# jmschrei/PyPore

Hardware: AMD Instinct MI355X
Metric: Msamples/sec segmented (SpeedyStatSplit, 10^8-sample trace); %HBM roofline (higher is better)
Workload: dtype int32/f64 (exact integer block sums of fp32 or int16 samples; decisions in fp64)

## Files before the change

### pypore_amd/csrc/seg_bs.hpp

```cpp
#pragma once
#include <type_traits>

namespace ps {

constexpr int BS_WIDE = 16384;
enum : unsigned { ST_WIDE_RANGE = 16u };
constexpr int BS_CHUNK = 128;
constexpr int BS_CHUNK_LOG = 7;
constexpr int BS_MAXCH = 64;
constexpr int BSW_LIM = 1 << 23;
template <int DT> constexpr bool bs_wide() { return (DT & DT_WIDE) != 0; }
__device__ __forceinline__ long long i64_of(int lo, int hi) { return (static_cast<long long>(hi) << 32) | static_cast<unsigned>(lo); }
__device__ __forceinline__ double d_of_i64(long long x)
{
    return fma(static_cast<double>(static_cast<int>(x >> 32)), 4294967296.0, static_cast<double>(static_cast<unsigned>(x)));
}
__device__ __forceinline__ unsigned long long u64_of(unsigned lo, unsigned hi) { return (static_cast<unsigned long long>(hi) << 32) | lo; }
__device__ __forceinline__ int bs8_s1(uint2 v) { return static_cast<int>(v.y) >> 7; }
__device__ __forceinline__ unsigned long long bs8_s2(uint2 v) { return u64_of(v.x, v.y & 0x7fu); }
__device__ __forceinline__ double bs8_s2_biased(uint2 v) { return __hiloint2double(static_cast<int>((v.y & 0x7fu) | 0x43300000u), static_cast<int>(v.x)); }
constexpr double BS_BIAS = 4503599627370496.0;
__device__ __forceinline__ uint2 bs8_pack(int e1, unsigned long long e2)
{
    return make_uint2(static_cast<unsigned>(e2), (static_cast<unsigned>(e1) << 7) | static_cast<unsigned>(e2 >> 32));
// ... 93 lines not shown
constexpr int BS_GRP_SAMPLES = 8 * BS_GRP;
#define PS_OCT_STEPS(X) X(0xB1) X(0x4E) X(0x141)
__device__ __forceinline__ int oct_allsum(int x)
{
#define PS_STEP(CTRL) { x += dpp_mov<CTRL, 0xf>(0, x); }
    PS_OCT_STEPS(PS_STEP)
#undef PS_STEP
    return x;
}
__device__ __forceinline__ int oct_allmax(int x)
{
#define PS_STEP(CTRL) { x = max(x, dpp_mov<CTRL, 0xf>(static_cast<int>(0x80000000), x)); }
    PS_OCT_STEPS(PS_STEP)
#undef PS_STEP
    return x;
}
__device__ __forceinline__ int oct_allmin(int x)
{
#define PS_STEP(CTRL) { x = min(x, dpp_mov<CTRL, 0xf>(0x7fffffff, x)); }
    PS_OCT_STEPS(PS_STEP)
#undef PS_STEP
    return x;
}
__device__ __forceinline__ float oct_allmaxf(float x)
{
#define PS_STEP(CTRL) { x = __uint_as_float(max(__float_as_uint(x), static_cast<unsigned>(dpp_mov<CTRL, 0xf>(0, static_cast<int>(__float_as_uint(x)))))); }
    PS_OCT_STEPS(PS_STEP)
#undef PS_STEP
    return x;
}
__device__ __forceinline__ float pmaxf(float a, float b) { return __int_as_float(max(__float_as_int(a), __float_as_int(b))); }
__device__ __forceinline__ int oct_first(int x, int lane)
{
    const int q = __builtin_amdgcn_update_dpp(0, x, 0x00, 0xf, 0xf, true);
    const int s = __builtin_amdgcn_update_dpp(0, q, 0x114, 0xf, 0xf, true);
    return (lane & 4) ? s : q;
}

#ifndef PS_K0_AMP
#define PS_K0_AMP 2
#endif
#ifndef PS_K0_TRIM
#define PS_K0_TRIM 1
#endif
#ifndef PS_K0_MINW
#define PS_K0_MINW 4
#endif
constexpr int K0_BPT = 4;
constexpr int K0_WB = 64 * K0_BPT;
#ifndef PS_K0_WAVES
#define PS_K0_WAVES 4
#endif
#ifndef PS_K0_PKF32
#define PS_K0_PKF32 1
#endif
#ifndef PS_K0_PK16
#define PS_K0_PK16 1
#endif
#ifndef PS_K0_PRIO
#define PS_K0_PRIO 0
#endif
constexpr int K0_WAVES = PS_K0_WAVES;
__host__ __device__ inline long long k0_padded_blocks(long long nb_total) { return (nb_total + 1 + K0_WB - 1) / K0_WB * K0_WB; }

__device__ __forceinline__ void k0_lds_ready() { asm volatile("s_waitcnt lgkmcnt(0)" ::: "memory"); __builtin_amdgcn_wave_barrier(); }
__device__ __forceinline__ void k0_lds_done() { __builtin_amdgcn_wave_barrier(); asm volatile("" ::: "memory"); }

template <int DT> struct K0Rec { int s1; unsigned s2; unsigned long long s2w; int ymin, ymax; };
template <int DT> struct K0Gen { K0Rec<DT> r; int m; unsigned bad; };

template <int DT>
__device__ __forceinline__ void k0_block_sums(const int (&y)[8], K0Rec<DT> &r)
{
    constexpr bool WIDE = bs_wide<DT>();
    r.s1 = 0; r.s2 = 0; r.s2w = 0;
#pragma unroll
    for (int q = 0; q < 8; ++q) {
        r.s1 += y[q];
        if constexpr (WIDE) r.s2w += static_cast<unsigned long long>(static_cast<long long>(y[q]) * static_cast<long long>(y[q]));
#if !PS_K0_TRIM
        else r.s2 += static_cast<unsigned>(__mul24(y[q], y[q]));
#endif
    }
#if PS_K0_TRIM
    if constexpr (!WIDE) {
        unsigned acc = static_cast<unsigned>(__mul24(y[0], y[0]));
#pragma unroll
        for (int q = 1; q < 8; ++q) asm("v_mad_i32_i24 %0, %1, %1, %2" : "=v"(acc) : "v"(y[q]), "v"(acc));
        r.s2 = acc;
    }
#endif
    r.ymin = min(min(min(y[0], y[1]), min(y[2], y[3])), min(min(y[4], y[5]), min(y[6], y[7])));
    r.ymax = max(max(max(y[0], y[1]), max(y[2], y[3])), max(max(y[4], y[5]), max(y[6], y[7])));
}

template <int DT>
__device__ __forceinline__ void k0_offsets(const DevCfg &c, const int4 *raw, int m, float mf, unsigned &nz, int (&y)[8])
{
    if (sdt(DT) == PS_DTYPE_F32) {
        const f2 iq = {c.inv_q, c.inv_q};
        const f2 mf2 = {mf, mf};
#pragma unroll
        for (int v = 0; v < 2; ++v) {
#pragma clang fp contract(off)
            const int w[4] = {raw[v].x, raw[v].y, raw[v].z, raw[v].w};
#pragma unroll
            for (int h = 0; h < 2; ++h) {
                const f2 x = {__int_as_float(w[2 * h]), __int_as_float(w[2 * h + 1])};
                const f2 t = x * iq;
                const f2 r = {__builtin_rintf(t.x), __builtin_rintf(t.y)};
                const f2 d = t - r;
                nz |= __float_as_uint(d.x) | __float_as_uint(d.y);
                const f2 yf = r - mf2;
                y[v * 4 + 2 * h] = static_cast<int>(yf.x);
                y[v * 4 + 2 * h + 1] = static_cast<int>(yf.y);
            }
        }
    } else {
        const int w[4] = {raw[0].x, raw[0].y, raw[0].z, raw[0].w};
        const int om = c.off_counts - m;
#pragma unroll
        for (int q = 0; q < 8; ++q)
            y[q] = ((q & 1) ? (w[q >> 1] >> 16) : static_cast<int>(static_cast<short>(w[q >> 1] & 0xffff))) + om;
    }
}

typedef short k0_v2s __attribute__((ext_vector_type(2)));
__device__ __forceinline__ int k0_dot2_first(k0_v2s a, k0_v2s b)
{
    int out;
    asm("v_dot2_i32_i16 %0, %1, %2, 0" : "=v"(out) : "v"(a), "v"(b));
    return out;
}

template <int DT>
__device__ __forceinline__ void k0_block_sums_pk16(const int4 raw, int k0pk, K0Rec<DT> &r)
{
    const k0_v2s k0v = __builtin_bit_cast(k0_v2s, k0pk);
    const k0_v2s ones = {1, 1};
    const int w[4] = {raw.x, raw.y, raw.z, raw.w};
    k0_v2s y[4];
    int s1 = 0, s2 = 0;
#pragma unroll
    for (int q = 0; q < 4; ++q) {
        y[q] = __builtin_elementwise_sub_sat(__builtin_bit_cast(k0_v2s, w[q]), k0v);
        s1 = q == 0 ? k0_dot2_first(y[q], ones) : __builtin_amdgcn_sdot2(y[q], ones, s1, false);
        s2 = q == 0 ? k0_dot2_first(y[q], y[q]) : __builtin_amdgcn_sdot2(y[q], y[q], s2, false);
    }
    const k0_v2s mn = __builtin_elementwise_min(__builtin_elementwise_min(y[0], y[1]), __builtin_elementwise_min(y[2], y[3]));
    const k0_v2s mx = __builtin_elementwise_max(__builtin_elementwise_max(y[0], y[1]), __builtin_elementwise_max(y[2], y[3]));
    r.s1 = s1; r.s2 = static_cast<unsigned>(s2); r.s2w = 0;
    r.ymin = min(static_cast<int>(mn.x), static_cast<int>(mn.y));
    r.ymax = max(static_cast<int>(mx.x), static_cast<int>(mx.y));
}

template <int DT>
__device__ __forceinline__ void k0_block_sums_pkf32(const int4 (&raw)[2], float inv_q, float mf, unsigned &nz, K0Rec<DT> &r)
{
    const f2 iq = {inv_q, inv_q}, m2 = {mf, mf};
    const f2 cn = {1.0f / 32767.0f, 1.0f / 32767.0f};
    const k0_v2s ones = {1, 1};
    const int w[8] = {raw[0].x, raw[0].y, raw[0].z, raw[0].w, raw[1].x, raw[1].y, raw[1].z, raw[1].w};
    k0_v2s y[4];
    int s1 = 0, s2 = 0;
#pragma unroll
    for (int h = 0; h < 4; ++h) {
#pragma clang fp contract(off)
        const f2 x = {__int_as_float(w[2 * h]), __int_as_float(w[2 * h + 1])};
        const f2 t = x * iq;
        nz |= __float_as_uint(__builtin_amdgcn_fractf(t.x)) | __float_as_uint(__builtin_amdgcn_fractf(t.y));
        const f2 a = (t - m2) * cn;
        y[h] = __builtin_amdgcn_cvt_pknorm_i16(a.x, a.y);
        s1 = h == 0 ? k0_dot2_first(y[h], ones) : __builtin_amdgcn_sdot2(y[h], ones, s1, false);
        s2 = h == 0 ? k0_dot2_first(y[h], y[h]) : __builtin_amdgcn_sdot2(y[h], y[h], s2, false);
    }
    const k0_v2s mn = __builtin_elementwise_min(__builtin_elementwise_min(y[0], y[1]), __builtin_elementwise_min(y[2], y[3]));
    const k0_v2s mx = __builtin_elementwise_max(__builtin_elementwise_max(y[0], y[1]), __builtin_elementwise_max(y[2], y[3]));
    r.s1 = s1; r.s2 = static_cast<unsigned>(s2); r.s2w = 0;
    r.ymin = min(static_cast<int>(mn.x), static_cast<int>(mn.y));
    r.ymax = max(static_cast<int>(mx.x), static_cast<int>(mx.y));
}

template <int DT>
__device__ __attribute__((noinline)) K0Gen<DT> k0_block_general(BsCold k, const int64_t *ev_start, const int64_t *ev_len, const int64_t *ev_boff,
                                                                int64_t n_samples, long long gb, long long nb_total, int e_hint, int4 *ev_info)
{
    const DevCfg c = bs_cold_cfg(k);
    K0Gen<DT> out;
    K0Rec<DT> &r = out.r;
    unsigned bad = 0;
    r.s1 = 0; r.s2 = 0; r.s2w = 0; r.ymin = 0; r.ymax = 0;
    out.m = 0; out.bad = 0;
    if (gb >= nb_total) return out;
    int e = e_hint;
    while (ev_boff[e + 1] <= gb) ++e;
    const int64_t len = ev_len[e], base = ev_start[e];
    const long long b = gb - ev_boff[e];
    const int64_t i0 = 8 * b;
    const int m = load_count<DT>(c, base, bad);
    out.m = m;
    int y[8];
    const int cnt = static_cast<int>(len - i0 < 8 ? len - i0 : 8);
    constexpr int ES = static_cast<int>(sizeof(typename Raw<DT>::type));
    const char *p = static_cast<const char *>(c.samples) + (base + i0) * ES;
    if (cnt == 8 && (reinterpret_cast<uintptr_t>(p) & 15u) == 0) {
        constexpr int NV = 8 * ES / 16;
        int4 raw[2];
#pragma unroll
        for (int v = 0; v < NV; ++v) raw[v] = reinterpret_cast<const int4 *>(p)[v];
        unsigned nz = 0;
        k0_offsets<DT>(c, raw, m, static_cast<float>(m), nz, y);
        if (nz) bad |= ST_OFF_GRID;
        k0_block_sums<DT>(y, r);
    } else if (sdt(DT) == PS_DTYPE_I16 && cnt == 8 && base + i0 >= 1 && base + i0 + 10 <= n_samples) {
        const uintptr_t a = reinterpret_cast<uintptr_t>(p);
        const int *q4 = reinterpret_cast<const int *>(a & ~static_cast<uintptr_t>(3));
        int v[5];
#pragma unroll
        for (int q = 0; q < 5; ++q) v[q] = q4[q];
        const bool odd = (a & 2u) != 0;
        const int om = c.off_counts - m;
#pragma unroll
        for (int q = 0; q < 4; ++q) {
            const int w = odd ? static_cast<int>((static_cast<unsigned>(v[q]) >> 16) | (static_cast<unsigned>(v[q + 1]) << 16)) : v[q];
            y[2 * q] = static_cast<int>(static_cast<short>(w & 0xffff)) + om;
            y[2 * q + 1] = (w >> 16) + om;
        }
        k0_block_sums<DT>(y, r);
    } else {
#pragma unroll
        for (int q = 0; q < 8; ++q) y[q] = q < cnt ? load_count<DT>(c, base + i0 + q, bad) - m : 0;
        k0_block_sums<DT>(y, r);
        r.ymin = r.ymax = y[0];
#pragma unroll
        for (int q = 1; q < 8; ++q)
            if (q < cnt) { r.ymin = min(r.ymin, y[q]); r.ymax = max(r.ymax, y[q]); }
    }
    if (b == 0) ev_info[e] = make_int4(m, 0, static_cast<int>(ev_boff[e] & 0xffffffffLL), static_cast<int>(ev_boff[e] >> 32));
    out.bad = bad;
    return out;
}

struct K0Src { int e; int fast; long long b_first; int64_t base; };
template <int A> struct K0Vec;
template <> struct K0Vec<2> { typedef int type __attribute__((ext_vector_type(4), aligned(2))); };
template <> struct K0Vec<4> { typedef int type __attribute__((ext_vector_type(4), aligned(4))); };
template <int A> __device__ __forceinline__ int4 k0_load16(const char *p)
{
    const typename K0Vec<A>::type v = *reinterpret_cast<const typename K0Vec<A>::type *>(p);
    return make_int4(v.x, v.y, v.z, v.w);
}
template <int A>
__global__ void k0_unaligned_probe_kernel(const unsigned char *buf, int n_off, unsigned *bad)
{
    const int o = threadIdx.x;
    if (o >= n_off) return;
    const int4 v = k0_load16<A>(reinterpret_cast<const char *>(buf) + o * A);
    const unsigned char *q = buf + o * A;
    unsigned w[4];
    for (int k = 0; k < 4; ++k) w[k] = q[4 * k] | (q[4 * k + 1] << 8) | (q[4 * k + 2] << 16) | (static_cast<unsigned>(q[4 * k + 3]) << 24);
    if (static_cast<unsigned>(v.x) != w[0] || static_cast<unsigned>(v.y) != w[1] || static_cast<unsigned>(v.z) != w[2] || static_cast<unsigned>(v.w) != w[3])
        atomicOr(bad, 1u);
}

template <int DT, int NS = 2>
__global__ __launch_bounds__(64 * K0_WAVES, (NS > 2 ? 2 : PS_K0_MINW)) void blocksum_kernel(DevCfg c, const int64_t *__restrict__ ev_start, const int64_t *__restrict__ ev_len,
                                                                const int64_t *__restrict__ ev_boff, int n_ev, int64_t n_samples, void *bs_out,
                                                                int4 *ev_info, int4 *chunk_tot, unsigned *status, uint4 *grp_out)
{
    constexpr bool WIDE = bs_wide<DT>();
    constexpr int LIM = WIDE ? BSW_LIM : BS_WIDE;
    constexpr int ES = static_cast<int>(sizeof(typename Raw<DT>::type));
    constexpr int NV = 8 * ES / 16;
    __shared__ int4 tr[K0_WAVES][K0_WB];
    const int lane = threadIdx.x & 63;
    const int wave = uni(static_cast<int>(threadIdx.x >> 6));
    const long long nwv = static_cast<long long>(gridDim.x) * K0_WAVES;
    long long wv = static_cast<long long>(blockIdx.x) * K0_WAVES + wave;
    const long long nb_total = ev_boff[n_ev];
    const long long n_wb = nb_total / K0_WB + 1;
    if (wv >= n_wb) return;
#if PS_K0_PRIO
    __builtin_amdgcn_s_setprio(PS_K0_PRIO);
#endif
    unsigned bad = 0;
    int4 *mine = tr[wave];
    auto classify = [&](long long wb0, int e_lo) -> K0Src {
        K0Src s;
        const long long gfirst = min(wb0, nb_total - 1);
        int lo = e_lo, hi = n_ev - 1;
        while (lo < hi) {
            const int mid = (lo + hi + 1) >> 1;
            if (ev_boff[mid] <= gfirst) lo = mid; else hi = mid - 1;
        }
        s.e = lo;
        s.b_first = wb0 - ev_boff[lo];
        s.base = ev_start[lo];
        const int64_t len_f = ev_len[lo];
        s.fast = wb0 + K0_WB <= ev_boff[lo + 1] && 8 * (s.b_first + K0_WB) <= len_f && nb_total > 0;
        if (!c.k0_unaligned && ((reinterpret_cast<uintptr_t>(c.samples) + static_cast<uintptr_t>((s.base + 8 * s.b_first) * ES)) & 15u) != 0) s.fast = 0;
        return s;
    };
    using raw_t = typename Raw<DT>::type;
    auto issue = [&](const K0Src &s, int4 (&raw)[K0_BPT][NV], raw_t &first) {
        const char *pb = s.fast ? static_cast<const char *>(c.samples) + (s.base + 8 * s.b_first) * ES : static_cast<const char *>(bs_out);
        first = *reinterpret_cast<const raw_t *>(s.fast ? static_cast<const char *>(c.samples) + s.base * ES : static_cast<const char *>(bs_out));
        const unsigned lo = static_cast<unsigned>(lane) * (8u * ES);
#pragma unroll
        for (int k = 0; k < K0_BPT; ++k)
#pragma unroll
            for (int v = 0; v < NV; ++v) raw[k][v] = k0_load16<ES>(pb + (lo + static_cast<unsigned>(k * 64 * 8 * ES + 16 * v)));
    };
    auto process = [&](auto fast_tag, const long long wb0, const K0Src &src, const int4 (&raw)[K0_BPT][NV], const raw_t first) {
    constexpr bool FAST = decltype(fast_tag)::value;
    const int e_first = src.e;
    int ymn_all = 0x7fffffff, ymx_all = -0x7fffffff - 1;
    auto put = [&](int k, const K0Rec<DT> &r) {
        if (PS_K0_TRIM) { ymn_all = min(ymn_all, r.ymin); ymx_all = max(ymx_all, r.ymax); }
        else if (r.ymax >= LIM || r.ymin <= -LIM) bad |= ST_WIDE_RANGE;
        if constexpr (WIDE) mine[64 * k + lane] = make_int4(r.s1, max(-r.ymin, r.ymax), static_cast<int>(r.s2w), static_cast<int>(r.s2w >> 32));
        else mine[64 * k + lane] = make_int4(r.s1, static_cast<int>(r.s2), (r.ymin & 0xffff) | (r.ymax << 16), 0);
    };
    if constexpr (FAST) {
        const int m = to_count<DT>(c, first, bad);
        const float mf = static_cast<float>(m);
        unsigned nz = 0;
        const bool look = sdt(DT) == PS_DTYPE_F32 && (WIDE || m > 8388607 - LIM || m < -8388607 + LIM);
        constexpr bool PK16 = sdt(DT) == PS_DTYPE_I16 && !WIDE && PS_K0_PK16;
        const int k0raw = m - c.off_counts;
        const int k0pk = (k0raw & 0xffff) | (k0raw << 16);
#pragma unroll
        for (int k = 0; k < K0_BPT; ++k) {
            int y[8];
            K0Rec<DT> r;
            if constexpr (PK16) {
                k0_block_sums_pk16<DT>(raw[k][0], k0pk, r);
            } else if constexpr (sdt(DT) == PS_DTYPE_F32 && !WIDE && PS_K0_PKF32) {
                k0_block_sums_pkf32<DT>(raw[k], c.inv_q, mf, nz, r);
                asm volatile("" : "+v"(nz));
            } else {
            k0_offsets<DT>(c, raw[k], m, mf, nz, y);
            asm volatile("" : "+v"(nz));
            k0_block_sums<DT>(y, r);
            }
            if (!PS_K0_TRIM && look) {
                const int ka = m + r.ymin, kb = m + r.ymax;
                if (max(ka < 0 ? -ka : ka, kb < 0 ? -kb : kb) >= 8388608) bad |= ST_OFF_GRID;
            }
            put(k, r);
            __builtin_amdgcn_sched_barrier(0);
        }
        if (PS_K0_TRIM && look) {
            const int ka = m + ymn_all, kb = m + ymx_all;
            if (max(ka < 0 ? -ka : ka, kb < 0 ? -kb : kb) >= 8388608) bad |= ST_OFF_GRID;
        }
        if (nz) bad |= ST_OFF_GRID;
        if (src.b_first + lane == 0) ev_info[e_first] = make_int4(m, 0, static_cast<int>(ev_boff[e_first] & 0xffffffffLL), static_cast<int>(ev_boff[e_first] >> 32));
    } else {
#pragma unroll 1
        for (int k = 0; k < K0_BPT; ++k) {
            const K0Gen<DT> g = k0_block_general<DT>(bs_cold(c), ev_start, ev_len, ev_boff, n_samples, wb0 + 64 * k + lane, nb_total, e_first, ev_info);
            bad |= g.bad;
            if (sdt(DT) == PS_DTYPE_F32) {
                const int ka = g.m + g.r.ymin, kb = g.m + g.r.ymax;
                if (max(ka < 0 ? -ka : ka, kb < 0 ? -kb : kb) >= 8388608) bad |= ST_OFF_GRID;
            }
            put(k, g.r);
        }
    }
    if (PS_K0_TRIM && (ymx_all >= LIM || ymn_all <= -LIM)) bad |= ST_WIDE_RANGE;
    k0_lds_ready();
    int4 t[K0_BPT];
#pragma unroll
    for (int j = 0; j < K0_BPT; ++j) t[j] = mine[K0_BPT * lane + j];
    const long long gb4 = wb0 + K0_BPT * lane;
    const long long chunk = (wb0 >> BS_CHUNK_LOG) + (lane >> 5);
    if constexpr (WIDE) {
        long long e1[K0_BPT], e2[K0_BPT];
        long long r1 = 0, r2 = 0;
        int yabs = 0;
#pragma unroll
        for (int j = 0; j < K0_BPT; ++j) {
            e1[j] = r1; e2[j] = r2;
            r1 += t[j].x; r2 += i64_of(t[j].z, t[j].w);
            yabs = max(yabs, t[j].y);
        }
        const long long i1 = half_incl_scan_i64(r1), i2 = half_incl_scan_i64(r2);
        const long long x1 = i1 - r1, x2 = i2 - r2;
        int4 *bs = static_cast<int4 *>(bs_out) + gb4;
#pragma unroll
        for (int j = 0; j < K0_BPT; ++j) {
            const long long a1 = x1 + e1[j], a2 = x2 + e2[j];
            bs[j] = make_int4(static_cast<int>(a1), static_cast<int>(a1 >> 32), static_cast<int>(a2), static_cast<int>(a2 >> 32));
        }
        yabs = half_max_i32(yabs);
        if ((lane & 31) == 31) {
            chunk_tot[2 * chunk] = make_int4(static_cast<int>(i1), static_cast<int>(i1 >> 32), static_cast<int>(i2), static_cast<int>(i2 >> 32));
            chunk_tot[2 * chunk + 1] = make_int4(yabs, 0, 0, 0);
        }
    } else {
        int e1[K0_BPT];
        unsigned long long e2[K0_BPT];
        int r1 = 0;
        unsigned long long r2 = 0;
#pragma unroll
        for (int j = 0; j < K0_BPT; ++j) {
            e1[j] = r1; e2[j] = r2;
            r1 += t[j].x; r2 += static_cast<unsigned>(t[j].y);
        }
        const int mmn = min(min(static_cast<int>(static_cast<short>(t[0].z & 0xffff)), static_cast<int>(static_cast<short>(t[1].z & 0xffff))),
                            min(static_cast<int>(static_cast<short>(t[2].z & 0xffff)), static_cast<int>(static_cast<short>(t[3].z & 0xffff))));
        const int mmx = max(max(t[0].z >> 16, t[1].z >> 16), max(t[2].z >> 16, t[3].z >> 16));
        int yabs = max(-mmn, mmx);
        const int i1 = half_incl_scan_i32(r1);
        const int r2lo = static_cast<int>(r2 & 0xffffu), r2hi = static_cast<int>(r2 >> 16);
        const int ilo = half_incl_scan_i32(r2lo), ihi = half_incl_scan_i32(r2hi);
        const int x1 = i1 - r1;
        const unsigned long long x2 = (static_cast<unsigned long long>(static_cast<unsigned>(ihi - r2hi)) << 16) + static_cast<unsigned>(ilo - r2lo);
        uint2 ent[K0_BPT];
#pragma unroll
        for (int j = 0; j < K0_BPT; ++j) ent[j] = bs8_pack(x1 + e1[j], x2 + e2[j]);
        uint4 *bs = reinterpret_cast<uint4 *>(static_cast<uint2 *>(bs_out) + gb4);
        bs[0] = make_uint4(ent[0].x, ent[0].y, ent[1].x, ent[1].y);
        bs[1] = make_uint4(ent[2].x, ent[2].y, ent[3].x, ent[3].y);
        if (c.blk_mm) *reinterpret_cast<int4 *>(c.blk_mm + gb4) = make_int4(t[0].z, t[1].z, t[2].z, t[3].z);
        if (c.blk_cls) {
            unsigned b2 = 0;
            const int ythr = c.cls_kthr - load_count<DT>(c, ev_start[0], b2);
            unsigned cb = 0;
            int cmn = 0x7fffffff, cmx = -0x7fffffff;
#pragma unroll
            for (int j = 0; j < K0_BPT; ++j) {
                const int lo_j = static_cast<int>(static_cast<short>(t[j].z & 0xffff)), hi_j = t[j].z >> 16;
                cb |= (hi_j < ythr ? 1u : lo_j >= ythr ? 0u : 2u) << (2 * j);
                if (gb4 + j < nb_total) { cmn = min(cmn, lo_j); cmx = max(cmx, hi_j); }
            }
            c.blk_cls[gb4 >> 2] = static_cast<unsigned char>(cb);
            cmn = -half_max_i32(-cmn);
            cmx = half_max_i32(cmx);
            if ((lane & 31) == 31) c.cls_mm[chunk] = make_int2(cmn, cmx);
        }
#if PS_K0_AMP == 2
        if (grp_out) {
            const int S1g = oct_allsum(r1);
            const double mg = static_cast<double>(S1g) * (-1.0 / 8192.0);
            float qf[K0_BPT];
#pragma unroll
            for (int j = 0; j < K0_BPT; ++j) {
                const int U = 64 * t[j].x - S1g;
                const float qx = static_cast<float>(fma(mg, static_cast<double>(U), static_cast<double>(static_cast<unsigned>(t[j].y))));
                qf[j] = PS_K0_TRIM ? __int_as_float(max(__float_as_int(qx), 0)) : fmaxf(qx, 0.0f);
            }
            const float lq = (qf[0] + qf[1]) + (qf[2] + qf[3]);
            float SSg = lq;
#define PS_STEP(CTRL) { SSg += dpp_movf<CTRL, 0xf>(0.0f, SSg); }
            PS_OCT_STEPS(PS_STEP)
#undef PS_STEP
            const float qbar = SSg * (1.0f / static_cast<float>(BS_GRP));
            const float lw = fmaf(-static_cast<float>(K0_BPT), qbar, lq);
            float inc = lw;
            const int l7 = lane & 7;
            { const float v = dpp_movf<0x111, 0xf>(0.0f, inc); inc += l7 >= 1 ? v : 0.0f; }
            { const float v = dpp_movf<0x112, 0xf>(0.0f, inc); inc += l7 >= 2 ? v : 0.0f; }
            { const float v = dpp_movf<0x114, 0xf>(0.0f, inc); inc += l7 >= 4 ? v : 0.0f; }
            float d2 = inc - lw;
            int p1 = x1 - oct_first(x1, lane);
            int nb = K0_BPT * l7;
            float a1p = fabsf(static_cast<float>(32 * p1 - nb * S1g)), a2p = fabsf(d2);
            float D1 = 0.0f, D2 = 0.0f;
#pragma unroll
            for (int j = 0; j < K0_BPT; ++j) {
                p1 += t[j].x; nb += 1;
                d2 += qf[j] - qbar;
                const float a1n = fabsf(static_cast<float>(32 * p1 - nb * S1g)), a2n = fabsf(d2);
#if PS_K0_TRIM
                D1 = pmaxf(D1, fmaf(pmaxf(a1p, a1n), 1.0f / 32.0f, __builtin_amdgcn_sqrtf(qf[j]) * 1.4142278f));
                D2 = pmaxf(D2, fmaf(0.875f, qf[j], pmaxf(a2p, a2n)));
#else
                D1 = fmaxf(D1, fmaf(fmaxf(a1p, a1n), 1.0f / 32.0f, __builtin_amdgcn_sqrtf(2.0f * qf[j]) * 1.00001f));
                D2 = fmaxf(D2, fmaf(0.875f, qf[j], fmaxf(a2p, a2n)));
#endif
                a1p = a1n; a2p = a2n;
            }
            D1 = oct_allmaxf(D1) * 1.00001f;
            D2 = fmaf(1.0e-5f, SSg, oct_allmaxf(D2) * 1.00001f);
            if (l7 == 0) grp_out[gb4 >> BS_GRP_LOG] = make_uint4(ent[0].x, ent[0].y, __float_as_uint(D1), __float_as_uint(D2));
        }
#else
        if (grp_out) {
            const int S1g = oct_allsum(r1);
            const int S2lo = oct_allsum(r2lo), S2hi = oct_allsum(r2hi);
            const double S2g = static_cast<double>(S2hi) * 65536.0 + static_cast<double>(S2lo);
            const int xlo = ilo - r2lo, xhi = ihi - r2hi;
            int p1 = x1 - oct_first(x1, lane);
            double p2 = static_cast<double>(xhi - oct_first(xhi, lane)) * 65536.0 + static_cast<double>(xlo - oct_first(xlo, lane));
            const double S1gd = static_cast<double>(S1g);
            const double k2 = S2g * (-1.0 / 32.0), k1 = S1gd * (-1.0 / 4096.0);
            const int jb0 = K0_BPT * (lane & 7);
            int m1 = 0;
            double m2 = 0.0;
#pragma unroll
            for (int j = 0; j < K0_BPT; ++j) {
                p1 += t[j].x;
                p2 += static_cast<double>(static_cast<unsigned>(t[j].y));
                const int jb = jb0 + j + 1;
                const int d1x = 32 * p1 - jb * S1g;
                const double d2 = fma(k1, static_cast<double>(d1x), fma(static_cast<double>(jb), k2, p2));
                m1 = max(m1, d1x < 0 ? -d1x : d1x);
                m2 = fmax(m2, fabs(d2));
            }
            const int gmn = oct_allmin(mmn), gmx = oct_allmax(mmx);
            m1 = oct_allmax(m1);
            const float m2f = oct_allmaxf(static_cast<float>(m2) * 1.000001f);
            const float mug = static_cast<float>(S1g) * (1.0f / static_cast<float>(BS_GRP_SAMPLES));
            const float Mg = fmaxf(static_cast<float>(gmx) - mug, mug - static_cast<float>(gmn)) * 1.000001f + 0.01f;
            const float D1 = (static_cast<float>(m1) * (1.0f / 32.0f) + 2.0f * static_cast<float>(gmx - gmn)) * 1.000001f;
            const float D2 = fmaf(2.0f * Mg, Mg, m2f) * 1.000001f;
            if ((lane & 7) == 0) grp_out[gb4 >> BS_GRP_LOG] = make_uint4(ent[0].x, ent[0].y, __float_as_uint(D1), __float_as_uint(D2));
        }
#endif
        yabs = half_max_i32(yabs);
        if ((lane & 31) == 31) {
            const unsigned long long tot2 = (static_cast<unsigned long long>(static_cast<unsigned>(ihi)) << 16) + static_cast<unsigned>(ilo);
            chunk_tot[chunk] = make_int4(i1, yabs, static_cast<int>(tot2), static_cast<int>(tot2 >> 32));
        }
    }
    k0_lds_done();
    };
    int4 raw[NS][K0_BPT][NV];
    raw_t first[NS];
    K0Src src[NS];
    unsigned long long general = 0;
    int it = 0;
    const long long wv0 = wv;
    auto retire = [&](const int4 (&rw)[K0_BPT][NV], const raw_t fs) {
#pragma unroll
        for (int k = 0; k < K0_BPT; ++k)
#pragma unroll
            for (int v = 0; v < NV; ++v) asm volatile("" :: "v"(rw[k][v].x), "v"(rw[k][v].y), "v"(rw[k][v].z), "v"(rw[k][v].w));
        asm volatile("" :: "v"(fs));
    };
    int e_hint = 0;
#pragma unroll
    for (int q = 0; q < NS - 1; ++q) {
        const long long wq = wv + q * nwv;
        if (wq < n_wb) { src[q] = classify(wq * K0_WB, e_hint); e_hint = src[q].e; }
        else { src[q] = src[0]; src[q].fast = 0; }
        issue(src[q], raw[q], first[q]);
    }
    bool last = false;
#pragma unroll 1
    while (!last) {
#pragma unroll
        for (int q = 0; q < NS; ++q) {
            if (last) break;
            constexpr int NSm1 = NS - 1;
            const int f = (q + NSm1) % NS;
            const long long wn = wv + static_cast<long long>(NSm1) * nwv;
            if (wn < n_wb) { src[f] = classify(wn * K0_WB, e_hint); e_hint = src[f].e; } else src[f].fast = 0;
            issue(src[f], raw[f], first[f]);
            if (src[q].fast) process(std::true_type{}, wv * K0_WB, src[q], raw[q], first[q]);
            else { general |= 1ull << min(it, 63); retire(raw[q], first[q]); }
            if (wv + nwv >= n_wb) last = true;
            else { wv += nwv; ++it; }
        }
    }
    if (general) {
        int e_lo = 0;
        it = 0;
#pragma unroll 1
        for (wv = wv0; wv < n_wb; wv += nwv, ++it) {
            if (it < 63 && !((general >> it) & 1ull)) continue;
            const K0Src sg = classify(wv * K0_WB, e_lo);
            e_lo = sg.e;
            if (!sg.fast) process(std::false_type{}, wv * K0_WB, sg, raw[0], first[0]);
        }
    }
    if (bad) atomicOr(status, bad);
}

struct BsEval { float g; f2 lg; f2 r; f2 u; bool okL, okR; };

__device__ __forceinline__ BsEval bs_eval(double a1d, double a2, double b1d, double b2, int nl, int nr, f2 cc, float vfloor)
{
    const double DL = fma(static_cast<double>(nl), a2, -(a1d * a1d));
    const double DR = fma(static_cast<double>(nr), b2, -(b1d * b1d));
    const f2 D = {static_cast<float>(DL), static_cast<float>(DR)};
    const f2 nv = {static_cast<float>(nl), static_cast<float>(nr)};
    const f2 r = {__builtin_amdgcn_rcpf(nv.x), __builtin_amdgcn_rcpf(nv.y)};
    const f2 u = D * r * r;
    const f2 lgu = {__builtin_amdgcn_logf(u.x), __builtin_amdgcn_logf(u.y)};
    BsEval o;
    o.lg = lgu - cc;
    o.r = r;
    o.u = u;
    o.okL = u.x >= vfloor;
    o.okR = u.y >= vfloor;
    const f2 t = nv * o.lg;
    o.g = -(t.x + t.y);
    return o;
}


__device__ __forceinline__ float bs_block_bound2(const BsEval &ep, const BsEval &eq, int p, int n, float SSt, float rn)
{
    const float LOG2E = 1.4426950408889634f;
    const float nf = static_cast<float>(n);
    const float pf = static_cast<float>(p), qf = pf + 8.0f, npf = nf - pf, nqf = npf - 8.0f;
    const float SSLp = pf * ep.u.x, SSRp = npf * ep.u.y, SSLq = qf * eq.u.x, SSRq = nqf * eq.u.y;
    const float eB = SSt * 2.0e-6f;
    const float Bp = (SSt - SSLp) - SSRp, Bq = (SSt - SSLq) - SSRq;
    const float Bpu = fmaxf(Bp, 0.0f) + eB, Bqu = fmaxf(Bq, 0.0f) + eB;
    const float DLb = fmaxf(SSLq - SSLp, 0.0f) + eB;
    const float Qb = fmaf(2.0f * fmaf(8.0f, ep.r.x, 1.0f), DLb, 16.0f * Bpu * (npf * rn) * ep.r.x);
    const float rK = __builtin_amdgcn_rcpf(fminf(pf * npf, qf * nqf));
    const float kap = fmaf(8.0f, fmaxf(ep.r.x, eq.r.y), 1.0f);
    const float sBQ = __builtin_amdgcn_sqrtf(fminf(Bpu, Bqu) * kap) + __builtin_amdgcn_sqrtf(7.0f * nf * Qb * rK);
    const float Bm = fmaf(sBQ, sBQ * 1.00001f, eB);
    const float s1 = fmaxf(Bm - (Bp - eB), 0.0f), s2 = fmaxf(Bm - (Bq - eB), 0.0f);
    const float v1 = fmaxf(SSRp - s1, SSRq), u2 = fmaxf(SSLq - s2, SSLp);
    const float e1 = (LOG2E * 1.00001f) * (SSRp - v1) * __builtin_amdgcn_rcpf(v1);
    const float e2 = (LOG2E * 1.00001f) * (SSLq - u2) * __builtin_amdgcn_rcpf(u2);
    const float Pp = ep.g + fmaf(7.0f, fabsf(ep.lg.x - ep.lg.y), (49.0f * LOG2E) * (ep.r.x + ep.r.y));
    const float Pq = eq.g + fmaf(7.0f, fabsf(eq.lg.x - eq.lg.y), (49.0f * LOG2E) * (eq.r.x + eq.r.y));
    const float hb = fmaxf(fmaf(npf, e1, Pp), fmaf(qf, e2, Pq)) + 1.0e-3f;
    const bool sound = static_cast<bool>(static_cast<int>(ep.okL) & static_cast<int>(ep.okR) & static_cast<int>(eq.okL) & static_cast<int>(eq.okR));
    return sound ? hb : INFINITY;
}

__device__ __forceinline__ float bs_group_slack(const BsEval &e, float D1, float D2, float wa, float wb, float dmu)
{
    const float LOG2E = 1.4426950408889634f;
    const float iVL = __builtin_amdgcn_rcpf(e.u.x), iVR = __builtin_amdgcn_rcpf(e.u.y);
    const float gS = iVL - iVR, dV = dmu * iVR;
    const float c1 = fmaxf(fabsf(fmaf(wa, gS, -dV)), fabsf(fmaf(wb, gS, -dV)));
    const float wL = fmaxf(fabsf(wa), fabsf(wb)), wR = fmaxf(fabsf(wa + dmu), fabsf(wb + dmu));
    const float D11 = D1 * D1;
    const float iSL = iVL * e.r.x, iSR = iVR * e.r.y;
    const float first = fmaf(D2, fabsf(gS), fmaf(2.0f * D1, c1, D11 * (iSL + iSR)));
    const float EL = fmaf(2.0f * wL, D1, fmaf(D11, e.r.x, D2)), ER = fmaf(2.0f * wR, D1, fmaf(D11, e.r.y, D2));
    const float tL = EL * iSL, tR = ER * iSR;
    const float second = fmaf(fmaf(0.44f, tL, 0.5f) * (EL * iVL), tL, fmaf(0.44f, tR, 0.5f) * (ER * iVR) * tR);
    const float A = fmaf((LOG2E * 1.0001f), first + second, 1.0e-3f);
    return (tL <= 0.3f && tR <= 0.3f) ? A : INFINITY;
}

struct BsQ { int j, a1; double a2; };
struct BsC { int j, a1; double a2; float g; int pad; };
struct BsQW { long long ja, a2; };
struct BsCW { int j; float g; long long a1, a2; };
static_assert(sizeof(BsQW) == sizeof(BsQ) && sizeof(BsCW) == sizeof(BsC), "LDS layout shared by both digests");
template <bool WIDE> struct BsTypes { typedef int s1_t; typedef double s2_t; typedef BsQ Q; typedef BsC C; typedef uint2 E; typedef double o2_t; };
template <> struct BsTypes<true> { typedef long long s1_t; typedef long long s2_t; typedef BsQW Q; typedef BsCW C; typedef int4 E; typedef long long o2_t; };
__device__ __forceinline__ double bs_d(int x) { return static_cast<double>(x); }
__device__ __forceinline__ double bs_d(double x) { return x; }
__device__ __forceinline__ double bs_d(long long x) { return d_of_i64(x); }
__device__ __forceinline__ void bs_q_put(BsQ &q, int J, int ps, int a1, double a2) { q.j = J; q.a1 = a1; q.a2 = a2; }
__device__ __forceinline__ void bs_q_put(BsQW &q, int J, int ps, long long a1, long long a2) { q.ja = a1 * 262144LL + (J - ps); q.a2 = a2; }
__device__ __forceinline__ int bs_q_j(const BsQ &q, int ps) { return q.j; }
__device__ __forceinline__ int bs_q_j(const BsQW &q, int ps) { return ps + static_cast<int>(q.ja & 262143LL); }
__device__ __forceinline__ int bs_q_a1(const BsQ &q) { return q.a1; }
__device__ __forceinline__ long long bs_q_a1(const BsQW &q) { return q.ja >> 18; }
__device__ __forceinline__ int bs_a1(uint2 e, int o1) { return bs8_s1(e) + o1; }
__device__ __forceinline__ double bs_a2(uint2 e, double k2) { return bs8_s2_biased(e) + k2; }
__device__ __forceinline__ long long bs_a1(const int4 &e, long long o1) { return i64_of(e.x, e.y) + o1; }
__device__ __forceinline__ long long bs_a2(const int4 &e, long long o2) { return i64_of(e.z, e.w) + o2; }
template <int DT>
__device__ __forceinline__ int bs_count_of(const DevCfg &c, typename Raw<DT>::type raw)
{
    if (sdt(DT) == PS_DTYPE_F32) return __float2int_rn(static_cast<float>(raw) * c.inv_q);
    return static_cast<int>(raw) + c.off_counts;
}
template <int DT>
__device__ __forceinline__ int bs_count(const DevCfg &c, int64_t gi)
{
    return bs_count_of<DT>(c, static_cast<const typename Raw<DT>::type *>(c.samples)[gi]);
}
constexpr int BS_NC = 64;
#ifndef PS_ONE_ROW_LOOP
#define PS_ONE_ROW_LOOP 0
#endif
#ifndef PS_RING_GUARD
#define PS_RING_GUARD 0
#endif
#ifndef PS_BS_D
#define PS_BS_D 2
#endif
constexpr int BS_D = PS_BS_D;
constexpr int BS_QN = 128;
#ifndef PS_DRAIN_FILTER
#define PS_DRAIN_FILTER 1
#endif
#ifndef PS_TREE_SAMPLE
#ifndef PS_ROW_OFFSETS_BPERMUTE
#define PS_ROW_OFFSETS_BPERMUTE 1
#endif
__device__ __forceinline__ int bs_from_lane(int x, int byte_index) { return __builtin_amdgcn_ds_bpermute(byte_index, x); }
__device__ __forceinline__ long long bs_from_lane(long long x, int byte_index)
{
    const int lo = __builtin_amdgcn_ds_bpermute(byte_index, static_cast<int>(x)), hi = __builtin_amdgcn_ds_bpermute(byte_index, static_cast<int>(x >> 32));
    return (static_cast<long long>(hi) << 32) | static_cast<unsigned>(lo);
}
__device__ __forceinline__ double bs_from_lane(double x, int byte_index) { return __longlong_as_double(bs_from_lane(__double_as_longlong(x), byte_index)); }
#define PS_TREE_SAMPLE 0
#endif
#ifndef PS_EDGE_PRELOAD
#define PS_EDGE_PRELOAD 1
#endif
constexpr int BS_EARLY = 64;
constexpr int BS_STRIDE = 63;
constexpr int BS_LDS_BYTES = (static_cast<int>(sizeof(BsQ)) + 8) * BS_QN + static_cast<int>(sizeof(BsC)) * BS_NC + 64 * 32;
static_assert(sizeof(QEnt) * SharedT<64>::QN >= BS_LDS_BYTES, "SharedT<64>::q too small");

__device__ __forceinline__ double bs_exact_gain(const DevCfg &c, int m, int a1, double a2, int T1, double T2, int nl, int n,
                                                double var_summed)
{
#pragma clang fp contract(off)
    const double dm = static_cast<double>(m);
    const double l1 = static_cast<double>(a1) + static_cast<double>(nl) * dm;
    const double l2 = a2 + 2.0 * dm * static_cast<double>(a1) + static_cast<double>(nl) * dm * dm;
    const int nr = n - nl;
    const int b1 = T1 - a1;
    const double b2 = T2 - a2;
    const double r1 = static_cast<double>(b1) + static_cast<double>(nr) * dm;
    const double r2 = b2 + 2.0 * dm * static_cast<double>(b1) + static_cast<double>(nr) * dm * dm;
    const double vl = ref_var(l1, l2, nl, c.q, c.q2), vr = ref_var(r1, r2, nr, c.q, c.q2);
    return ref_gain(var_summed, nl, vl, nr, vr);
}

__device__ __forceinline__ int lanes_below(unsigned long long mask)
{
    return __builtin_amdgcn_mbcnt_hi(static_cast<unsigned>(mask >> 32), __builtin_amdgcn_mbcnt_lo(static_cast<unsigned>(mask), 0u));
}
__device__ __forceinline__ int from_lane_below(int x) { return __builtin_amdgcn_update_dpp(x, x, 0x138, 0xf, 0xf, false); }
__device__ __forceinline__ float from_lane_below(float x) { return __int_as_float(from_lane_below(__float_as_int(x))); }
__device__ __forceinline__ int from_lane_above(int x) { return __builtin_amdgcn_update_dpp(x, x, 0x130, 0xf, 0xf, false); }
__device__ __forceinline__ float from_lane_above(float x) { return __int_as_float(from_lane_above(__float_as_int(x))); }
__device__ __forceinline__ int oct_sum(int x)
{
    x += dpp_mov<0x111, 0xf>(0, x); x += dpp_mov<0x112, 0xf>(0, x); x += dpp_mov<0x114, 0xf>(0, x);
    return x;
}
__device__ __forceinline__ long long oct_sum(long long x)
{
#define PS_STEP(CTRL) { const int lo_ = dpp_mov<CTRL, 0xf>(0, static_cast<int>(x)), hi_ = dpp_mov<CTRL, 0xf>(0, static_cast<int>(x >> 32)); x += i64_of(lo_, hi_); }
    PS_STEP(0x111) PS_STEP(0x112) PS_STEP(0x114)
#undef PS_STEP
    return x;
}

template <int DT>
__device__ __attribute__((noinline)) long long bs_scan_exact(BsCold k, int64_t g0, int ps, int n, int cand_lo, int cand_hi,
                                                             double thresh, SharedT<64> *sh)
{
    const DevCfg c = bs_cold_cfg(k);
    unsigned bad = 0;
    const int r = scan_exact<64, DT>(c, nullptr, g0, ps, n, cand_lo, cand_hi, thresh, nullptr, *sh, bad, nullptr);
    return (static_cast<long long>(bad) << 32) | static_cast<unsigned>(r);
}

struct BsDecideCold { const NtLog *lg; double q, q2, dc_counts; float noise_k; };
__device__ __forceinline__ BsDecideCold bs_decide_cold(const DevCfg &c) { BsDecideCold k = {c.nt_log, c.q, c.q2, c.dc_counts, c.noise_k}; return k; }
template <int DT>
__device__ __attribute__((noinline)) long long bs_decide(BsDecideCold k, int m, const void *cont_v, int ccount, int ps, int n,
                                                         typename BsTypes<bs_wide<DT>()>::s1_t T1, typename BsTypes<bs_wide<DT>()>::s2_t T2,
                                                         double thresh, long long g0)
{
    DevCfg cfg = {};
    cfg.q = k.q; cfg.q2 = k.q2;
    const DevCfg *c = &cfg;
    const NtLog *lg = k.lg;
    int near = 0;
    constexpr bool WIDE = bs_wide<DT>();
    typedef typename BsTypes<WIDE>::C BsC_t;
    const BsC_t *cont = static_cast<const BsC_t *>(cont_v);
    const int lane = threadIdx.x & 63;
    const double T1d = bs_d(T1), T2d = bs_d(T2), dn = static_cast<double>(n);
    double var_summed;
    if constexpr (WIDE) var_summed = dn * log(ref_var(T1d, T2d, n, c->q, c->q2));
    else var_summed = dn * log(ref_var(T1d + dn * static_cast<double>(m),
                                       T2d + 2.0 * static_cast<double>(m) * T1d + dn * static_cast<double>(m) * static_cast<double>(m), n, c->q, c->q2));
    double eg = thresh;
    int ei = -1;
    double gx = -INFINITY;
    double noise = 0.0, noise_tot = 0.0;
    const double nk = static_cast<double>(k.noise_k);
    if (lane < ccount) {
        const BsC_t e = cont[lane];
        if constexpr (WIDE) {
            const int nl = e.j - ps;
            const double vl = ref_var(d_of_i64(e.a1), d_of_i64(e.a2), nl, c->q, c->q2);
            const double vr = ref_var(d_of_i64(T1 - e.a1), d_of_i64(T2 - e.a2), n - nl, c->q, c->q2);
            gx = ref_gain(var_summed, nl, vl, n - nl, vr);
            const double vt = ref_var(T1d, T2d, n, c->q, c->q2);
            const double lvl = (fabs(k.dc_counts + static_cast<double>(m)) + sqrt(fmax(vt, 0.0) / c->q2)) * c->q;
            const double ulp2 = static_cast<double>(ps + n) * lvl * lvl * 2.220446049250313e-16;
            const double tiny = 1.0e-300;
            auto part = [&](int np, double vp) {
                const double sn = sqrt(static_cast<double>(np));
                return ulp2 * sn * 0.2887 / fmax(vp, tiny) + 0.6 * sn * c->q / sqrt(fmax(vp, tiny));
            };
            noise = part(nl, vl) + part(n - nl, vr);
            noise_tot = part(n, vt);
        } else {
            gx = bs_exact_gain(*c, m, e.a1, e.a2, T1, T2, e.j - ps, n, var_summed);
        }
        if (gx > eg) { eg = gx; ei = e.j; }
    }
#pragma unroll
    for (int d = 32; d >= 1; d >>= 1) {
        const double og = __shfl_xor(eg, d);
        const int oi = __shfl_xor(ei, d);
        if (beats(og, oi, eg, ei)) { eg = og; ei = oi; }
    }
    if (ei >= 0) {
        double other = (lane < ccount && cont[lane].j != ei) ? gx : -INFINITY;
        if (!(other == other)) other = -INFINITY;
#pragma unroll
        for (int d = 32; d >= 1; d >>= 1) other = fmax(other, __shfl_xor(other, d));
        const double tol = 1.0e-9 * fmax(1.0, fabs(eg));
        near = (eg - other < tol || eg - thresh < tol) ? 1 : 0;
        if constexpr (WIDE) {
            double nw = (lane < ccount && cont[lane].j == ei) ? noise : 0.0;
#pragma unroll
            for (int d = 32; d >= 1; d >>= 1) nw = fmax(nw, __shfl_xor(nw, d));
            const bool mine = lane < ccount && cont[lane].j != ei && gx == gx && eg - gx < nk * (nw + noise);
            const bool thr_near = eg - thresh < nk * (nw + __shfl(noise_tot, 0));
            if (__ballot(mine) != 0ull || thr_near) near = 1;
        }
    } else {
        double best = (lane < ccount && gx == gx) ? gx : -INFINITY;
#pragma unroll
        for (int d = 32; d >= 1; d >>= 1) best = fmax(best, __shfl_xor(best, d));
        const double tol = 1.0e-9 * fmax(1.0, fabs(thresh));
        near = thresh - best < tol ? 1 : 0;
        if constexpr (WIDE) {
            const bool mine = lane < ccount && gx == gx && thresh - gx < nk * (noise + noise_tot);
            if (__ballot(mine) != 0ull) near = 1;
        }
    }
    if (near && lg && lane == 0) {
        const unsigned long long slot = atomicAdd(lg->cur, 1ull);
        if (slot < static_cast<unsigned long long>(lg->cap)) {
            NtRec r;
            r.start = g0; r.len = n; r.split = ei >= 0 ? ei - ps : -1;
            const_cast<NtLog *>(lg)->rec[slot] = r;
        }
    }
    return (static_cast<long long>(near) << 32) | static_cast<unsigned>(ei);
}

__device__ __forceinline__ void bs_audit_note(unsigned long long *a, int icnt, int iviol, int imin, float bound, float gmax, float tol)
{
    if (!(bound < INFINITY)) return;
    atomicAdd(&a[icnt], 1ull);
    if (gmax == -INFINITY) return;
    const float margin = bound - gmax;
    if (!(margin >= -tol)) atomicAdd(&a[iviol], 1ull);
    int k = __float_as_int(margin);
    k ^= (k >> 31) & 0x7fffffff;
    atomicMin(reinterpret_cast<int *>(&a[imin]), k);
}

#ifdef PS_MARKS
#define PS_MARK(n) asm volatile("; PSMARK " #n)
#else
#define PS_MARK(n) do { } while (0)
#endif

struct BsGeom {
    int n, g0, g1, nblk, gbl, nch, rows, nh, nt;
    long long gb0, G0;
    __device__ __forceinline__ bool off_path(int cand_lo, int cand_hi) const { return nblk < 4 || nch > BS_MAXCH || cand_lo < g0 || cand_hi > g1; }
    __device__ __forceinline__ int whole_groups() const { return min(static_cast<int>(((gb0 + nblk) >> BS_GRP_LOG) - G0), 63); }
};
__device__ __forceinline__ BsGeom bs_geom(const EvRef &er, int ps, int pe)
{
    BsGeom g;
// ... 841 lines not shown
```

Before: 544,800.

## Deepen K0 load pipeline to NS stages and split process into sums and tail

The kernel now prefetches all NS slots up front and splits per-tile processing into a register-only sums phase and an LDS scan tail. The refill load for a slot is issued between them, fenced by sched_barriers, so global loads overlap the LDS scan work. It also narrows the first-sample load for int16 to a 2-byte-aligned unsigned and uses two base pointers with an SGPR hop to cut address arithmetic. This raises register pressure, since more raw buffers are live, and the loop-exit logic changes in ways that could affect the general-path bookkeeping.

Measured after the change: 543,800 (median of 3 runs). About the same (-0.2%).

```diff
diff --git a/pypore_amd/csrc/seg_bs.hpp b/pypore_amd/csrc/seg_bs.hpp
--- a/pypore_amd/csrc/seg_bs.hpp
+++ b/pypore_amd/csrc/seg_bs.hpp
@@ -419,17 +419,26 @@
         return s;
     };
     using raw_t = typename Raw<DT>::type;
-    auto issue = [&](const K0Src &s, int4 (&raw)[K0_BPT][NV], raw_t &first) {
+    typedef unsigned k0_first_i16 __attribute__((aligned(2)));
+    using first_t = std::conditional_t<sdt(DT) == PS_DTYPE_I16, unsigned, raw_t>;
+    using first_ld = std::conditional_t<sdt(DT) == PS_DTYPE_I16, k0_first_i16, raw_t>;
+    auto issue = [&](const K0Src &s, int4 (&raw)[K0_BPT][NV], first_t &first) {
         const char *pb = s.fast ? static_cast<const char *>(c.samples) + (s.base + 8 * s.b_first) * ES : static_cast<const char *>(bs_out);
-        first = *reinterpret_cast<const raw_t *>(s.fast ? static_cast<const char *>(c.samples) + s.base * ES : static_cast<const char *>(bs_out));
-        const unsigned lo = static_cast<unsigned>(lane) * (8u * ES);
+        unsigned fz = 0;
+        if (sdt(DT) == PS_DTYPE_I16) asm("" : "+v"(fz));
+        first = *reinterpret_cast<const first_ld *>((s.fast ? static_cast<const char *>(c.samples) + s.base * ES : static_cast<const char *>(bs_out)) + fz);
+        const unsigned lo = static_cast<unsigned>(lane) * (s.fast ? 8u * ES : 0u);
+        long long hop = 2 * 64 * 8 * ES;
+        asm("" : "+s"(hop));
+        const char *pbh[2] = {pb, pb + hop};
 #pragma unroll
         for (int k = 0; k < K0_BPT; ++k)
 #pragma unroll
-            for (int v = 0; v < NV; ++v) raw[k][v] = k0_load16<ES>(pb + (lo + static_cast<unsigned>(k * 64 * 8 * ES + 16 * v)));
+            for (int v = 0; v < NV; ++v) raw[k][v] = k0_load16<ES>(pbh[k >> 1] + ((k & 1) * 64 * 8 * ES + 16 * v) + lo);
     };
-    auto process = [&](auto fast_tag, const long long wb0, const K0Src &src, const int4 (&raw)[K0_BPT][NV], const raw_t first) {
+    auto sums = [&](auto fast_tag, const long long wb0, const K0Src &src, const int4 (&raw)[K0_BPT][NV], const first_t first_bits) {
     constexpr bool FAST = decltype(fast_tag)::value;
+    const raw_t first = static_cast<raw_t>(static_cast<std::conditional_t<sdt(DT) == PS_DTYPE_I16, unsigned short, raw_t>>(first_bits));
     const int e_first = src.e;
     int ymn_all = 0x7fffffff, ymx_all = -0x7fffffff - 1;
     auto put = [&](int k, const K0Rec<DT> &r) {
@@ -486,6 +495,8 @@
         }
     }
     if (PS_K0_TRIM && (ymx_all >= LIM || ymn_all <= -LIM)) bad |= ST_WIDE_RANGE;
+    };
+    auto tail = [&](const long long wb0) {
     k0_lds_ready();
     int4 t[K0_BPT];
 #pragma unroll
@@ -645,12 +656,12 @@
     k0_lds_done();
     };
     int4 raw[NS][K0_BPT][NV];
-    raw_t first[NS];
+    first_t first[NS];
     K0Src src[NS];
     unsigned long long general = 0;
     int it = 0;
     const long long wv0 = wv;
-    auto retire = [&](const int4 (&rw)[K0_BPT][NV], const raw_t fs) {
+    auto retire = [&](const int4 (&rw)[K0_BPT][NV], const first_t fs) {
 #pragma unroll
         for (int k = 0; k < K0_BPT; ++k)
 #pragma unroll
@@ -659,29 +670,29 @@
     };
     int e_hint = 0;
 #pragma unroll
-    for (int q = 0; q < NS - 1; ++q) {
+    for (int q = 0; q < NS; ++q) {
         const long long wq = wv + q * nwv;
         if (wq < n_wb) { src[q] = classify(wq * K0_WB, e_hint); e_hint = src[q].e; }
         else { src[q] = src[0]; src[q].fast = 0; }
         issue(src[q], raw[q], first[q]);
     }
-    bool last = false;
 #pragma unroll 1
-    while (!last) {
+    do {
 #pragma unroll
         for (int q = 0; q < NS; ++q) {
-            if (last) break;
-            constexpr int NSm1 = NS - 1;
-            const int f = (q + NSm1) % NS;
-            const long long wn = wv + static_cast<long long>(NSm1) * nwv;
-            if (wn < n_wb) { src[f] = classify(wn * K0_WB, e_hint); e_hint = src[f].e; } else src[f].fast = 0;
-            issue(src[f], raw[f], first[f]);
-            if (src[q].fast) process(std::true_type{}, wv * K0_WB, src[q], raw[q], first[q]);
-            else { general |= 1ull << min(it, 63); retire(raw[q], first[q]); }
-            if (wv + nwv >= n_wb) last = true;
-            else { wv += nwv; ++it; }
-        }
-    }
+            const long long wb0 = wv * K0_WB;
+            const bool fast = src[q].fast != 0;
+            if (fast) sums(std::true_type{}, wb0, src[q], raw[q], first[q]);
+            else { if (wv < n_wb) general |= 1ull << min(it, 63); retire(raw[q], first[q]); }
+            __builtin_amdgcn_sched_barrier(0);
+            const long long wn = wv + static_cast<long long>(NS) * nwv;
+            if (wn < n_wb) { src[q] = classify(wn * K0_WB, e_hint); e_hint = src[q].e; } else src[q].fast = 0;
+            issue(src[q], raw[q], first[q]);
+            __builtin_amdgcn_sched_barrier(0);
+            if (fast) tail(wb0);
+            wv += nwv; ++it;
+        }
+    } while (wv < n_wb);
     if (general) {
         int e_lo = 0;
         it = 0;
@@ -690,7 +701,7 @@
             if (it < 63 && !((general >> it) & 1ull)) continue;
             const K0Src sg = classify(wv * K0_WB, e_lo);
             e_lo = sg.e;
-            if (!sg.fast) process(std::false_type{}, wv * K0_WB, sg, raw[0], first[0]);
+            if (!sg.fast) { sums(std::false_type{}, wv * K0_WB, sg, raw[0], first[0]); tail(wv * K0_WB); }
         }
     }
     if (bad) atomicOr(status, bad);
```
